# andrenarchy/krypy

Hardware: AMD Instinct MI355X
Metric: GMRES iterations/sec + SpMV HBM GB/s, n=10^7 5-pt Laplacian fp64 (higher is better)
Workload: dtype f64; 1 GPU; GMRES(100) restart cycles, 2-D 5-pt Laplacian 4000x2500 CSR (N=10000000, nnz=49987000), b=rng(0) normal, x0=0, tol=1e-8 (BASELINE.json configs[1]); n=10000000, ortho=mgs, restart=100, parallelism=1 GPU, ranks=1

## Files before the change

krypy_amd/csrc/chain.h:

```cpp
#pragma once
#include <type_traits>
#include "kernels.h"

namespace kh {

constexpr int CH_BS = 512;
constexpr int CH_GMAX = 512;

struct ChainArgs {
    int64_t n2;
    int64_t chunk2;
    const double* V;
    const double* B;
    int64_t ld;
    int64_t col0;
    int ncol;
    int sweeps;
    const double* w_in;
    const double* dg;
    double* vnext;
    double* pnext;
    double* hdev;
    int64_t hnext;
    unsigned long long* gran;
// ... 631 lines not shown
#pragma unroll
    for (int d = 0; d < FND; ++d) {
#pragma unroll
        for (int p = 0; p < 2; ++p) {
            const int o = a.offs.off[d] + p;
            kq[d][p] = (unsigned)((o >> 1) - g.lo * CH_BS);
            kh[d][p] = (o & 1) ? H : 0u;
        }
    }
    {
        const int64_t b0 = first + (int64_t)g.lo * CH_BS;
        constexpr int PG = 8;
#pragma unroll
        for (int j0 = 0; j0 < NWB - 1; j0 += PG) {
            double2 t[PG];
#pragma unroll
            for (int j = j0; j < j0 + PG && j < NWB - 1; ++j) t[j - j0] = xw.load(b0 + (int64_t)(j < spanb ? j : spanb - 1) * CH_BS);
            CH_ISSUE_FENCE();
#pragma unroll
            for (int j = j0; j < j0 + PG && j < NWB - 1; ++j) xw.store((unsigned)j, tid, t[j - j0]);
        }
    }
    double2 st[D];
    unsigned mk[D];
    int64_t fb = first;
    const int64_t hs = (int64_t)(g.hi + 1) * CH_BS;
#pragma unroll
    for (int r = 0; r < D; ++r) {
        mk[r] = dia_mask_load(a.dmask, fb + (int64_t)r * CH_BS);
        st[r] = xw.load(fb + hs + (int64_t)r * CH_BS);
    }
    unsigned sl = (unsigned)spanb;
    unsigned tb = (unsigned)tid;
    ch_lds_barrier();
#pragma unroll
    for (int r = 0; r < R2; ++r) {
        const unsigned m = mk[r % D];
        const unsigned pos = (unsigned)((r % NWB) * CH_BS) + tb;
        double2 av[FND];
        double x0[FND], x1[FND];
#pragma unroll
        for (int d = 0; d < FND; ++d) {
            av[d] = dia_slot<true>(a.dia, a.dia_ld, d, 0, m, a.offs.cst[d]);
            x0[d] = xw.get(pos, kq[d][0], kh[d][0]);
            x1[d] = xw.get(pos, kq[d][1], kh[d][1]);
        }
        double s0 = 0.0, s1 = 0.0;
#pragma unroll
        for (int d = 0; d < FND; ++d) {
            const double p0 = av[d].x * x0[d], p1 = av[d].y * x1[d];
            s0 = (av[d].x != 0.0) ? s0 + p0 : s0;
            s1 = (av[d].y != 0.0) ? s1 + p1 : s1;
        }
        put(r, s0, s1);
        if (r + 1 < R2) {
            xw.store(sl, tid, st[r % D]);
            sl = (sl + 1 == (unsigned)NWB) ? 0u : sl + 1;
        }
        if (r + D < R2) mk[r % D] = dia_mask_load(a.dmask, fb + (int64_t)(r + D) * CH_BS);
        if (r + D + 1 < R2) st[r % D] = xw.load(fb + hs + (int64_t)(r + D) * CH_BS);
        ch_lds_barrier();
        asm volatile("" : "+v"(fb), "+v"(tb) : : "memory");
    }
}

template <int R2, int FND, int RIF = KH_RIF, class Put>
__device__ __forceinline__ void chain_apply_banded(const ChainArgs& a, int64_t first, Put&& put) {
    static_assert(FND <= KH_DIA_CMAX, "the mask form holds up to KH_DIA_CMAX diagonals");
    if (a.dmask != nullptr) chain_apply_banded_form<R2, FND, RIF, true>(a, first, put);
    else chain_apply_banded_form<R2, FND, RIF, false>(a, first, put);
}

template <int R2, bool MASKED, bool CPLX = false, int FND = 0, int WL = 0, bool ONEX = false, bool XR = false>
__global__ __launch_bounds__(CH_BS) void k_mgs_chain(ChainArgs a) {
    static_assert(FND == 0 || !MASKED, "the fused operator exists for the padded kernels");
    static_assert(!XR || (!CPLX && !ONEX), "the cross-rank stage exists for real vectors spread over the chip");
    constexpr int RW = R2 - WL;
    extern __shared__ __attribute__((aligned(16))) double2 wl[];
#define W_GET(r) (((r) < RW) ? w[((r) < RW) ? (r) : 0] : wl[((r) - RW) * CH_BS + tid])
#define W_PUT(r, val)                                   \
    do {                                                \
        if ((r) < RW) w[((r) < RW) ? (r) : 0] = (val);  \
        else wl[((r) - RW) * CH_BS + tid] = (val);      \
    } while (0)
    constexpr int PB = ChainShape<R2>::PB;
    constexpr int NB = ChainShape<R2>::NB;
    __shared__ double smd[4 * (CH_BS / 64)];
    __shared__ unsigned smu[2 * CH_GMAX];
    __shared__ int slead;
    const int tid = threadIdx.x;
    int G = gridDim.x;
    int bid = blockIdx.x;
    GridRole role;
    if constexpr (ONEX) {
        if (!onex_enter(a, &slead, bid, G, role)) return;
    } else {
        role = grid_role(a.xcc_leader, a.epoch0, &slead);
    }
    const int64_t first = (int64_t)bid * a.chunk2 + tid;
    const int64_t left = a.n2 - first;
    const int rem = (int)(left < 0 ? 0 : (left > a.chunk2 ? a.chunk2 : left));
#define CH_OK(r) (!MASKED || (r) * CH_BS < rem)
    double2 w[RW];
    double2 ring[2][PB];
    if constexpr (FND > 0 && CPLX) {
        chain_apply_banded_z<R2, FND>(a, first, [&](int r, double s0, double s1) { W_PUT(r, make_double2(s0, s1)); });
    } else if constexpr (FND > 0) {
        chain_apply_banded<R2, FND>(a, first, [&](int r, double s0, double s1) { W_PUT(r, make_double2(s0, s1)); });
    } else {
        const double2* __restrict__ win2 = reinterpret_cast<const double2*>(a.w_in) + first;
#pragma unroll
        for (int r = 0; r < R2; ++r) {
            const double2 v = win2[(int64_t)r * CH_BS];
            double2 t;
            t.x = CH_OK(r) ? v.x : 0.0;
            t.y = CH_OK(r) ? v.y : 0.0;
            W_PUT(r, t);
            if ((r + 1) % 8 == 0) CH_ISSUE_FENCE();
        }
    }
    if (a.presub) {
        const double hk = (a.h_km1_dev != nullptr) ? a.h_km1_dev[0] : a.h_km1;
        const double2* __restrict__ p2 = reinterpret_cast<const double2*>(a.bprev) + first;
#pragma unroll
        for (int r = 0; r < R2; ++r) {
            const double2 p = p2[(int64_t)r * CH_BS];
            double2 t = W_GET(r);
            t.x = CH_OK(r) ? t.x - hk * p.x : 0.0;
            t.y = CH_OK(r) ? t.y - hk * p.y : 0.0;
            W_PUT(r, t);
            if ((r + 1) % 8 == 0) CH_ISSUE_FENCE();
        }
    }
    unsigned epoch = a.epoch0;
    if (a.debug == 4 && tid == 0) __hip_atomic_store(a.err, 1, __ATOMIC_RELAXED, __HIP_MEMORY_SCOPE_AGENT);
    const int total = a.ncol * a.sweeps;
    {
        const double2* __restrict__ v2 = reinterpret_cast<const double2*>(a.V + a.col0 * a.ld) + first;
#pragma unroll
        for (int i = 0; i < PB; ++i) ring[0][i] = v2[(int64_t)i * CH_BS];
        CH_ISSUE_FENCE();
    }
    for (int t = 0; t < total; ++t) {
        const int64_t j = a.col0 + (t % a.ncol);
        const double2* __restrict__ v2 = reinterpret_cast<const double2*>(a.V + j * a.ld) + first;
        const double2* __restrict__ b2 = reinterpret_cast<const double2*>(a.B + j * a.ld) + first;
        double acc0 = 0.0, acc1 = 0.0;
        if (a.debug != 2)
#pragma unroll
        for (int b = 0; b < NB; ++b) {
            const double2* __restrict__ nx = (b + 1 < NB) ? v2 + (int64_t)(b + 1) * PB * CH_BS : b2;
#pragma unroll
            for (int i = 0; i < PB; ++i)
                ring[(b + 1) & 1][i] = (WL > 0 && b + 1 == NB) ? ld_nt2(nx + (int64_t)i * CH_BS) : nx[(int64_t)i * CH_BS];
            CH_ISSUE_FENCE();
#pragma unroll
            for (int i = 0; i < PB; ++i) {
                double2 v = ring[b & 1][i];
                if (MASKED && !CH_OK(b * PB + i)) v = make_double2(0.0, 0.0);
                const double2 wr = W_GET(b * PB + i);
                if (CPLX) {
                    acc0 = fma(v.x, wr.x, acc0);
                    acc0 = fma(v.y, wr.y, acc0);
                    acc1 = fma(v.x, wr.y, acc1);
                    acc1 = fma(-v.y, wr.x, acc1);
                } else {
                    acc0 = fma(v.x, wr.x, acc0);
                    acc1 = fma(v.y, wr.y, acc1);
                }
            }
        }
        double alpha, alpha_i = 0.0;
        if (CPLX) {
            alpha = acc0;
            alpha_i = acc1;
            if constexpr (ONEX) {
                double pv[2] = {alpha, alpha_i};
                onex_sum<2>(pv, epoch++, a.gran, G, bid, a.err, smd);
                alpha = pv[0];
                alpha_i = pv[1];
            } else {
                grid_sum2(alpha, alpha_i, epoch++, a.gran, G, a.err, smd, smu, role, a.xcc_res);
            }
            if (bid == 0 && tid == 0) {
                a.hdev[2 * j] = (t < a.ncol ? 0.0 : a.hdev[2 * j]) + alpha;
                a.hdev[2 * j + 1] = (t < a.ncol ? 0.0 : a.hdev[2 * j + 1]) + alpha_i;
            }
        } else {
            if constexpr (ONEX) {
                double pv[1] = {acc0 + acc1};
                onex_sum<1>(pv, epoch++, a.gran, G, bid, a.err, smd);
                alpha = pv[0];
            } else {
                const unsigned e_ = epoch++;
                alpha = (a.debug == 1) ? (acc0 + acc1) * 1e-30
                                       : grid_sum<XR>(acc0 + acc1, e_, a.gran, G, a.err, smd, smu, role, a.xcc_res, nullptr, &a.xr,
                                                      a.xr.epoch0 + (e_ - a.epoch0));
            }
            if (bid == 0 && tid == 0) a.hdev[j] = (t < a.ncol ? 0.0 : a.hdev[j]) + alpha;
        }
        if (a.debug == 4) alpha *= 0.5;
        const int64_t jn = a.col0 + ((t + 1) % a.ncol);
        const double2* __restrict__ vn = (t + 1 < total)
            ? reinterpret_cast<const double2*>(a.V + jn * a.ld) + first
            : reinterpret_cast<const double2*>(a.w_in) + first;
        if (a.debug != 2)
#pragma unroll
        for (int b = 0; b < NB; ++b) {
            const double2* __restrict__ nx = (b + 1 < NB) ? b2 + (int64_t)(b + 1) * PB * CH_BS : vn;
#pragma unroll
            for (int i = 0; i < PB; ++i)
                ring[(b + 1) & 1][i] = (WL > 0 && b + 1 < NB) ? ld_nt2(nx + (int64_t)i * CH_BS) : nx[(int64_t)i * CH_BS];
            CH_ISSUE_FENCE();
#pragma unroll
            for (int i = 0; i < PB; ++i) {
                const double2 p = ring[b & 1][i];
                const int r = b * PB + i;
                double2 wr = W_GET(r);
                if (CPLX) {
                    const double tr = alpha * p.x - alpha_i * p.y;
                    const double ti = alpha * p.y + alpha_i * p.x;
                    wr.x = CH_OK(r) ? wr.x - tr : 0.0;
                    wr.y = CH_OK(r) ? wr.y - ti : 0.0;
                } else {
                    wr.x = CH_OK(r) ? wr.x - alpha * p.x : 0.0;
                    wr.y = CH_OK(r) ? wr.y - alpha * p.y : 0.0;
                }
                W_PUT(r, wr);
            }
        }
    }
    double acc = 0.0;
    if (a.dg != nullptr) {
        const double2* __restrict__ d2 = reinterpret_cast<const double2*>(a.dg) + first;
#pragma unroll
        for (int r = 0; r < R2; ++r) {
            const double2 d = d2[(int64_t)r * CH_BS];
            const double2 wr = W_GET(r);
            acc = fma(wr.x, d.x * wr.x, acc);
            acc = fma(wr.y, d.y * wr.y, acc);
            if ((r + 1) % 8 == 0) CH_ISSUE_FENCE();
        }
    } else {
#pragma unroll
        for (int r = 0; r < R2; ++r) {
            const double2 wr = W_GET(r);
            acc = fma(wr.x, wr.x, acc);
            acc = fma(wr.y, wr.y, acc);
        }
    }
    double h2;
    if constexpr (ONEX) {
        double pv[1] = {acc};
        onex_sum<1>(pv, epoch++, a.gran, G, bid, a.err, smd);
        h2 = pv[0];
    } else {
        const unsigned e_ = epoch++;
        h2 = grid_sum<XR>(acc, e_, a.gran, G, a.err, smd, smu, role, a.xcc_res, nullptr, &a.xr, a.xr.epoch0 + (e_ - a.epoch0));
    }
    const double h = sqrt(fabs(h2));
    if (bid == 0 && tid == 0) a.hdev[a.hnext] = h;
    double2* __restrict__ vn2 = reinterpret_cast<double2*>(a.vnext) + first;
    if (a.dg != nullptr) {
        double2* __restrict__ pn2 = reinterpret_cast<double2*>(a.pnext) + first;
        const double2* __restrict__ d2 = reinterpret_cast<const double2*>(a.dg) + first;
#pragma unroll
        for (int r = 0; r < R2; ++r) {
            if (r * CH_BS < rem) {
                const double2 d = d2[(int64_t)r * CH_BS];
                const double2 wr = W_GET(r);
                double2 o, m;
                o.x = wr.x / h;
                o.y = wr.y / h;
                m.x = (d.x * wr.x) / h;
                m.y = (d.y * wr.y) / h;
                st_nt2(pn2 + (int64_t)r * CH_BS, o);
                st_nt2(vn2 + (int64_t)r * CH_BS, m);
            }
        }
    } else {
#pragma unroll
        for (int r = 0; r < R2; ++r) {
            if (r * CH_BS < rem) {
                const double2 wr = W_GET(r);
                double2 o;
                o.x = wr.x / h;
                o.y = wr.y / h;
                st_nt2(vn2 + (int64_t)r * CH_BS, o);
            }
        }
    }
    if (bid == 0 && a.hpin != nullptr) {
        __syncthreads();
        for (int i = tid; i < a.hcount; i += CH_BS)
            a.hpin[i] = __hip_atomic_load(a.hdev + i, __ATOMIC_RELAXED, __HIP_MEMORY_SCOPE_AGENT);
        if (tid == 0) *a.errpin = __hip_atomic_load(a.err, __ATOMIC_RELAXED, __HIP_MEMORY_SCOPE_AGENT);
        CH_SIGNAL_DONE(a);
    }
#undef W_PUT
#undef W_GET
#undef CH_OK
}

#ifndef KH_CH_REUSE_SKIP
#define KH_CH_REUSE_SKIP 0
#endif
#ifndef KH_CH_SKIP_LAST
#define KH_CH_SKIP_LAST 0
#endif
#ifndef KH_CH_LDS_EARLY
#define KH_CH_LDS_EARLY 0
#endif
#ifndef KH_XWIN_AHEAD
#define KH_XWIN_AHEAD 4
#endif
template <int R2, bool CPLX = false>
struct ChainShapeLds {
    static constexpr int PB = ChainShape<R2>::PB;
    static constexpr int NB = R2 / PB;
    static constexpr int WL = (R2 == 40 && !CPLX) ? 4 : 0;
    static constexpr int LROWS = (R2 == 40 && !CPLX) ? 19 : (NB >= 4 ? 3 : 1) * PB;
    static constexpr int NG = NB - 1 - LROWS / PB;
    static_assert((NB % 2) == 0 && NG >= 0 && (NG % 2) == 0, "ring parity must reset every phase");
    static_assert(WL <= LROWS && LROWS <= R2 - PB, "the prologue's rows of w borrow parked rows; the last batch stays in the ring");
    static constexpr size_t LDS_BYTES = (size_t)LROWS * CH_BS * sizeof(double2);
    static constexpr int XWIN_BLOCKS = LROWS - WL;
    static constexpr size_t STATIC_LDS = 4 * (CH_BS / 64) * sizeof(double) + 2 * CH_GMAX * sizeof(unsigned) + sizeof(int);
    static_assert(LDS_BYTES + STATIC_LDS <= 160 * 1024, "a CU has 160 KB of LDS");
};

template <int R2, bool MASKED, bool CPLX = false, int FND = 0, bool XR = false>
__global__ __launch_bounds__(CH_BS) void k_mgs_chain_lds(ChainArgs a) {
    static_assert(FND == 0 || !MASKED, "the fused operator exists for the padded kernels");
    static_assert(!XR || !CPLX, "the cross-rank stage exists for real vectors");
    constexpr int PB = ChainShapeLds<R2, CPLX>::PB;
    constexpr int NB = ChainShapeLds<R2, CPLX>::NB;
    constexpr int LROWS = ChainShapeLds<R2, CPLX>::LROWS;
    constexpr int LBC = (LROWS + PB - 1) / PB;
    constexpr bool SPLIT = (LROWS % PB) != 0;
    constexpr int NG = ChainShapeLds<R2, CPLX>::NG;
    constexpr int WL = FND > 0 ? ChainShapeLds<R2, CPLX>::WL : 0;
    constexpr int RW = R2 - WL;
    extern __shared__ __attribute__((aligned(16))) double2 vlds[];
#define W_GET_N(r, NR) (((r) < (NR)) ? w[((r) < (NR)) ? (r) : 0] : vlds[((r) - (NR)) * CH_BS + tid])
#define W_PUT_N(r, val, NR)                                 \
    do {                                                    \
        if ((r) < (NR)) w[((r) < (NR)) ? (r) : 0] = (val);  \
        else vlds[((r) - (NR)) * CH_BS + tid] = (val);      \
    } while (0)
#define W_GET(r) W_GET_N(r, RW)
#define W_PUT(r, val) W_PUT_N(r, val, RW)
    __shared__ double smd[4 * (CH_BS / 64)];
    __shared__ unsigned smu[2 * CH_GMAX];
    __shared__ int slead;
    const int tid = threadIdx.x;
    const int G = gridDim.x;
    const GridRole role = grid_role(a.xcc_leader, a.epoch0, &slead);
    const int64_t first = (int64_t)blockIdx.x * a.chunk2 + tid;
    const int64_t left = a.n2 - first;
    const int rem = (int)(left < 0 ? 0 : (left > a.chunk2 ? a.chunk2 : left));
#define CH_OK(r) (!MASKED || (r) * CH_BS < rem)
#define CH_LD(ptr, reuse) ((reuse) ? *(ptr) : ld_nt2(ptr))
    double2 w[R2];
    double2 ring[2][PB];
    if constexpr (FND > 0 && CPLX) {
        chain_apply_banded_z<R2, FND>(a, first, [&](int r, double s0, double s1) { W_PUT(r, make_double2(s0, s1)); });
    } else if constexpr (FND > 0 && !XR) {
        constexpr int NWB = ChainShapeLds<R2, CPLX>::XWIN_BLOCKS;
        if (a.xwin)
            chain_apply_banded_xwin<R2, FND, NWB, KH_XWIN_AHEAD>(a, first, reinterpret_cast<double*>(vlds + WL * CH_BS),
                                                                 [&](int r, double s0, double s1) { W_PUT(r, make_double2(s0, s1)); });
        else
            chain_apply_banded<R2, FND>(a, first, [&](int r, double s0, double s1) { W_PUT(r, make_double2(s0, s1)); });
    } else if constexpr (FND > 0) {
        chain_apply_banded<R2, FND>(a, first, [&](int r, double s0, double s1) { W_PUT(r, make_double2(s0, s1)); });
    } else {
        const double2* __restrict__ win2 = reinterpret_cast<const double2*>(a.w_in) + first;
#pragma unroll
        for (int r = 0; r < R2; ++r) {
            const double2 v = ld_nt2(win2 + (int64_t)r * CH_BS);
            double2 t;
            t.x = CH_OK(r) ? v.x : 0.0;
            t.y = CH_OK(r) ? v.y : 0.0;
            W_PUT(r, t);
            if ((r + 1) % 8 == 0) CH_ISSUE_FENCE();
        }
    }
    if (a.presub) {
        const double hk = (a.h_km1_dev != nullptr) ? a.h_km1_dev[0] : a.h_km1;
        const double2* __restrict__ p2 = reinterpret_cast<const double2*>(a.bprev) + first;
#pragma unroll
        for (int r = 0; r < R2; ++r) {
            const double2 p = p2[(int64_t)r * CH_BS];
            double2 t = W_GET(r);
            t.x = CH_OK(r) ? t.x - hk * p.x : 0.0;
            t.y = CH_OK(r) ? t.y - hk * p.y : 0.0;
            W_PUT(r, t);
            if ((r + 1) % 8 == 0) CH_ISSUE_FENCE();
        }
    }
    if constexpr (WL > 0) {
#pragma unroll
        for (int r = RW; r < R2; ++r) w[r] = vlds[(r - RW) * CH_BS + tid];
        CH_ISSUE_FENCE();
    }
#undef W_PUT
#undef W_GET
#define W_GET(r) W_GET_N(r, R2)
#define W_PUT(r, val) W_PUT_N(r, val, R2)
    unsigned epoch = a.epoch0;
    if (a.debug == 4 && tid == 0) __hip_atomic_store(a.err, 1, __ATOMIC_RELAXED, __HIP_MEMORY_SCOPE_AGENT);
    const int total = a.ncol * a.sweeps;
    {
        const double2* __restrict__ v2 = reinterpret_cast<const double2*>(a.V + a.col0 * a.ld) + first;
#pragma unroll
        for (int i = 0; i < PB; ++i) ring[0][i] = CH_LD(v2 + (int64_t)i * CH_BS, false);
        CH_ISSUE_FENCE();
    }
#if defined(KH_CHAIN_TRACE) && KH_CHAIN_TRACE == 2
    unsigned long long tr_acc[9] = {0, 0, 0, 0, 0, 0, 0, 0, 0};
#endif
    for (int t = 0; t < total; ++t) {
        const int64_t j = a.col0 + (t % a.ncol);
        const double2* __restrict__ v2 = reinterpret_cast<const double2*>(a.V + j * a.ld) + first;
        const int64_t jn = a.col0 + ((t + 1) % a.ncol);
        const double2* __restrict__ vn = (t + 1 < total)
            ? reinterpret_cast<const double2*>(a.V + jn * a.ld) + first
            : reinterpret_cast<const double2*>(a.w_in) + first;
        double acc0 = 0.0, acc1 = 0.0;
        CH_STAMP(a, t, total, 0);
#pragma unroll
        for (int b = 0; b < NB; ++b) {
            const double2* __restrict__ nx = (b + 1 < NB) ? v2 + (int64_t)(b + 1) * PB * CH_BS
                                                            : (NG > 0 ? v2 + (int64_t)(NB - 2) * PB * CH_BS : vn);
#pragma unroll
            for (int i = 0; i < PB; ++i) {
                if (!SPLIT || b + 1 < NB || NG == 0 || (NB - 2) * PB + i >= LROWS)
                    ring[(b + 1) & 1][i] = CH_LD(nx + (int64_t)i * CH_BS, (b + 1 < NB) && (!SPLIT || (b + 1) * PB + i >= LROWS) &&
                                                                              (b + 1 >= LROWS / PB + KH_CH_REUSE_SKIP) && (b + 1 <= NB - 2 - KH_CH_SKIP_LAST));
            }
            CH_ISSUE_FENCE();
#pragma unroll
            for (int i = 0; i < PB; ++i) {
                double2 v = ring[b & 1][i];
                if (MASKED && !CH_OK(b * PB + i)) v = make_double2(0.0, 0.0);
                if (SPLIT ? (b * PB + i < LROWS) : (b < LBC)) vlds[(b * PB + i) * CH_BS + tid] = v;
                const double2 wr = W_GET(b * PB + i);
                if (CPLX) {
                    acc0 = fma(v.x, wr.x, acc0);
                    acc0 = fma(v.y, wr.y, acc0);
                    acc1 = fma(v.x, wr.y, acc1);
                    acc1 = fma(-v.y, wr.x, acc1);
                } else {
                    acc0 = fma(v.x, wr.x, acc0);
                    acc1 = fma(v.y, wr.y, acc1);
                }
            }
        }
        double alpha, alpha_i = 0.0;
        CH_STAMP(a, t, total, 1);
        if (CPLX) {
            alpha = acc0;
            alpha_i = acc1;
            grid_sum2(alpha, alpha_i, epoch++, a.gran, G, a.err, smd, smu, role, a.xcc_res);
            if (blockIdx.x == 0 && tid == 0) {
                a.hdev[2 * j] = (t < a.ncol ? 0.0 : a.hdev[2 * j]) + alpha;
                a.hdev[2 * j + 1] = (t < a.ncol ? 0.0 : a.hdev[2 * j + 1]) + alpha_i;
            }
        } else {
#if defined(KH_CHAIN_TRACE) && KH_CHAIN_TRACE == 2
            alpha = grid_sum(acc0 + acc1, epoch++, a.gran, G, a.err, smd, smu, role, a.xcc_res, tr_acc);
#elif defined(KH_CHAIN_TRACE)
            alpha = grid_sum(acc0 + acc1, epoch++, a.gran, G, a.err, smd, smu, role, a.xcc_res,
                             a.trace ? a.trace + (((size_t)blockIdx.x * total) + t) * 16 : nullptr);
#else
            const unsigned e_ = epoch++;
            alpha = (a.debug == 1) ? (acc0 + acc1) * 1e-30
                                   : grid_sum<XR>(acc0 + acc1, e_, a.gran, G, a.err, smd, smu, role, a.xcc_res, nullptr, &a.xr,
                                                  a.xr.epoch0 + (e_ - a.epoch0));
#endif
            if (blockIdx.x == 0 && tid == 0) a.hdev[j] = (t < a.ncol ? 0.0 : a.hdev[j]) + alpha;
        }
        if (a.debug == 4) alpha *= 0.5;
        CH_STAMP(a, t, total, 5);
#define CH_UPD(r, p)                                              \
    do {                                                          \
        double2 wr_ = W_GET(r);                                   \
        if (CPLX) {                                               \
            const double tr = alpha * (p).x - alpha_i * (p).y;    \
            const double ti = alpha * (p).y + alpha_i * (p).x;    \
            wr_.x = CH_OK(r) ? wr_.x - tr : 0.0;                  \
            wr_.y = CH_OK(r) ? wr_.y - ti : 0.0;                  \
        } else {                                                  \
            wr_.x = CH_OK(r) ? wr_.x - alpha * (p).x : 0.0;       \
            wr_.y = CH_OK(r) ? wr_.y - alpha * (p).y : 0.0;       \
        }                                                         \
        W_PUT(r, wr_);                                            \
    } while (0)
#pragma unroll
        for (int i = 0; i < PB; ++i) CH_UPD((NB - 1) * PB + i, ring[1][i]);
        constexpr bool EARLY = (KH_CH_LDS_EARLY != 0) && NG >= 2;
#pragma unroll
        for (int g = 0; g < NG; ++g) {
            const int b = NB - 2 - g;
            const double2* __restrict__ nx = (g + 1 < NG) ? v2 + (int64_t)(b - 1) * PB * CH_BS : vn;
#pragma unroll
            for (int i = 0; i < PB; ++i) {
                if (!SPLIT || g + 1 == NG || (b - 1) * PB + i >= LROWS) ring[(g + 1) & 1][i] = CH_LD(nx + (int64_t)i * CH_BS, false);
            }
            CH_ISSUE_FENCE();
            if (EARLY && g == 1) {
#pragma unroll
                for (int bb = LBC - 1; bb >= 0; --bb) {
#pragma unroll
                    for (int i = 0; i < PB; ++i) {
                        if (!SPLIT || bb * PB + i < LROWS) {
                            const double2 p = vlds[(bb * PB + i) * CH_BS + tid];
                            CH_UPD(bb * PB + i, p);
                        }
                    }
                    CH_ISSUE_FENCE();
                }
            }
#pragma unroll
            for (int i = 0; i < PB; ++i) {
                if (!SPLIT || b * PB + i >= LROWS) CH_UPD(b * PB + i, ring[g & 1][i]);
            }
        }
        CH_STAMP(a, t, total, 6);
        if (!EARLY) {
#pragma unroll
            for (int b = LBC - 1; b >= 0; --b) {
                CH_ISSUE_FENCE();
#pragma unroll
                for (int i = 0; i < PB; ++i) {
                    if (!SPLIT || b * PB + i < LROWS) {
                        const double2 p = vlds[(b * PB + i) * CH_BS + tid];
                        CH_UPD(b * PB + i, p);
                    }
                }
            }
        }
#undef CH_UPD
        CH_STAMP(a, t, total, 7);
    }
#if defined(KH_CHAIN_TRACE) && KH_CHAIN_TRACE == 2
    if (a.trace != nullptr && (tid == 0 || tid == CH_BS - 64)) {
#pragma unroll
        for (int i = 0; i < 8; ++i) a.trace[((size_t)blockIdx.x * 2 + (tid ? 1 : 0)) * 8 + i] = tr_acc[i];
    }
#endif
    double acc = 0.0;
    if (a.dg != nullptr) {
        const double2* __restrict__ d2 = reinterpret_cast<const double2*>(a.dg) + first;
#pragma unroll
        for (int r = 0; r < R2; ++r) {
            const double2 d = d2[(int64_t)r * CH_BS];
            const double2 wr = W_GET(r);
            acc = fma(wr.x, d.x * wr.x, acc);
            acc = fma(wr.y, d.y * wr.y, acc);
            if ((r + 1) % 8 == 0) CH_ISSUE_FENCE();
        }
    } else {
#pragma unroll
        for (int r = 0; r < R2; ++r) {
            const double2 wr = W_GET(r);
            acc = fma(wr.x, wr.x, acc);
            acc = fma(wr.y, wr.y, acc);
        }
    }
    const unsigned en_ = epoch++;
    const double h2 = grid_sum<XR>(acc, en_, a.gran, G, a.err, smd, smu, role, a.xcc_res, nullptr, &a.xr, a.xr.epoch0 + (en_ - a.epoch0));
    const double h = sqrt(fabs(h2));
    if (blockIdx.x == 0 && tid == 0) a.hdev[a.hnext] = h;
    double2* __restrict__ vn2 = reinterpret_cast<double2*>(a.vnext) + first;
    if (a.dg != nullptr) {
        double2* __restrict__ pn2 = reinterpret_cast<double2*>(a.pnext) + first;
        const double2* __restrict__ d2 = reinterpret_cast<const double2*>(a.dg) + first;
#pragma unroll
        for (int r = 0; r < R2; ++r) {
            if (r * CH_BS < rem) {
                const double2 d = d2[(int64_t)r * CH_BS];
                const double2 wr = W_GET(r);
                double2 o, m;
                o.x = wr.x / h;
                o.y = wr.y / h;
                m.x = (d.x * wr.x) / h;
                m.y = (d.y * wr.y) / h;
                st_nt2(pn2 + (int64_t)r * CH_BS, o);
                st_nt2(vn2 + (int64_t)r * CH_BS, m);
            }
        }
    } else {
#pragma unroll
        for (int r = 0; r < R2; ++r) {
            if (r * CH_BS < rem) {
                const double2 wr = W_GET(r);
                double2 o;
                o.x = wr.x / h;
                o.y = wr.y / h;
                st_nt2(vn2 + (int64_t)r * CH_BS, o);
            }
        }
    }
    if (blockIdx.x == 0 && a.hpin != nullptr) {
        __syncthreads();
        for (int i = tid; i < a.hcount; i += CH_BS)
            a.hpin[i] = __hip_atomic_load(a.hdev + i, __ATOMIC_RELAXED, __HIP_MEMORY_SCOPE_AGENT);
        if (tid == 0) *a.errpin = __hip_atomic_load(a.err, __ATOMIC_RELAXED, __HIP_MEMORY_SCOPE_AGENT);
        CH_SIGNAL_DONE(a);
    }
#undef W_PUT
#undef W_GET
#undef W_PUT_N
#undef W_GET_N
#undef CH_LD
#undef CH_OK
}

template <int R2>
struct ChainShapePf {
    static constexpr int PB = ChainShape<R2>::PB;
    static constexpr int NB = R2 / PB;
    static constexpr int LB = (NB - 2 < 3) ? NB - 2 : 3;
    static constexpr int NG = NB - 2 - LB;
    static_assert((NB % 2) == 0 && NB >= 2 && LB >= 0 && NG >= 0 && NG <= LB, "shape");
    static constexpr int ROW_BYTES = CH_BS * (int)sizeof(double2);
    static constexpr int STATIC_LDS = 2 * (CH_BS / 64) * 8 + 2 * CH_GMAX * 4 + 256;
    static constexpr int SPARE = (160 * 1024 - STATIC_LDS - LB * PB * ROW_BYTES) / ROW_BYTES;
#ifndef KH_PF_SP_CAP
#define KH_PF_SP_CAP 64
#endif
    static constexpr int SP0 = SPARE < PB ? SPARE : PB;
    static constexpr int SP = SP0 < KH_PF_SP_CAP ? SP0 : KH_PF_SP_CAP;
    static_assert(SP0 >= 1, "at least one spare row");
    static constexpr size_t LDS_BYTES = (size_t)(LB * PB + SP) * ROW_BYTES;
};

typedef __attribute__((address_space(3))) double2 ch_lds_double2;

__device__ __forceinline__ void ch_dma16(const double2* gsrc, unsigned lds_dst) {
    unsigned keep;
    asm volatile("s_mov_b32 %0, m0\n\ts_mov_b32 m0, %2\n\ts_nop 0\n\tglobal_load_lds_dwordx4 %1, off\n\ts_mov_b32 m0, %0"
                 : "=&s"(keep)
                 : "v"(gsrc), "s"(lds_dst)
                 : "memory");
}

template <int R2, bool MASKED, bool CPLX = false, int FND = 0, bool ONEX = false>
__global__ __launch_bounds__(CH_BS) void k_mgs_chain_pf(ChainArgs a) {
    static_assert(FND == 0 || (!MASKED && !CPLX), "the fused operator exists for the padded real kernel");
    constexpr int PB = ChainShapePf<R2>::PB;
    constexpr int NB = ChainShapePf<R2>::NB;
    constexpr int LB = ChainShapePf<R2>::LB;
    constexpr int NG = ChainShapePf<R2>::NG;
    constexpr int SP = ChainShapePf<R2>::SP;
    extern __shared__ __attribute__((aligned(16))) double2 vlds[];
    double2* const vsp = vlds + (size_t)LB * PB * CH_BS;
    __shared__ double smd[4 * (CH_BS / 64)];
    __shared__ unsigned smu[2 * CH_GMAX];
    __shared__ int slead;
    const int tid = threadIdx.x;
    int G = gridDim.x;
    int bid = blockIdx.x;
    GridRole role;
    if constexpr (ONEX) {
        if (!onex_enter(a, &slead, bid, G, role)) return;
    } else {
        role = grid_role(a.xcc_leader, a.epoch0, &slead);
    }
    const int64_t first = (int64_t)bid * a.chunk2 + tid;
    const int64_t left = a.n2 - first;
    const int rem = (int)(left < 0 ? 0 : (left > a.chunk2 ? a.chunk2 : left));
    const unsigned lds_wave = (unsigned)(size_t)((ch_lds_double2*)vlds) +
                              (unsigned)__builtin_amdgcn_readfirstlane((tid >> 6) * 64 * (int)sizeof(double2));
#define CH_OK(r) (!MASKED || (r) * CH_BS < rem)
#define CH_LD(ptr, reuse) ((reuse) ? *(ptr) : ld_nt2(ptr))
    double2 w[R2];
    double2 ring[2][PB];
    if constexpr (FND > 0) {
        chain_apply_banded<R2, FND>(a, first, [&](int r, double s0, double s1) { w[r] = make_double2(s0, s1); });
    } else {
        const double2* __restrict__ win2 = reinterpret_cast<const double2*>(a.w_in) + first;
#pragma unroll
        for (int r = 0; r < R2; ++r) {
            const double2 v = ld_nt2(win2 + (int64_t)r * CH_BS);
            w[r].x = CH_OK(r) ? v.x : 0.0;
            w[r].y = CH_OK(r) ? v.y : 0.0;
            if ((r + 1) % 8 == 0) CH_ISSUE_FENCE();
        }
    }
    if (a.presub) {
        const double hk = (a.h_km1_dev != nullptr) ? a.h_km1_dev[0] : a.h_km1;
        const double2* __restrict__ p2 = reinterpret_cast<const double2*>(a.bprev) + first;
#pragma unroll
        for (int r = 0; r < R2; ++r) {
            const double2 p = p2[(int64_t)r * CH_BS];
            w[r].x = CH_OK(r) ? w[r].x - hk * p.x : 0.0;
            w[r].y = CH_OK(r) ? w[r].y - hk * p.y : 0.0;
            if ((r + 1) % 8 == 0) CH_ISSUE_FENCE();
        }
    }
    unsigned epoch = a.epoch0;
    if (a.debug == 4 && tid == 0) __hip_atomic_store(a.err, 1, __ATOMIC_RELAXED, __HIP_MEMORY_SCOPE_AGENT);
    const int total = a.ncol * a.sweeps;
#define CH_REUSE(b) ((b) >= LB && (b) < LB + NG)
    {
        const double2* __restrict__ v2 = reinterpret_cast<const double2*>(a.V + a.col0 * a.ld) + first;
#pragma unroll
        for (int i = 0; i < SP; ++i)
            ch_dma16(v2 + (int64_t)i * CH_BS, lds_wave + (unsigned)(((LB * PB + i) * CH_BS) * sizeof(double2)));
#pragma unroll
        for (int i = SP; i < PB; ++i) ring[0][i] = CH_LD(v2 + (int64_t)i * CH_BS, CH_REUSE(0));
        CH_ISSUE_FENCE();
        if (NB > 1) {
#pragma unroll
            for (int i = 0; i < PB; ++i) ring[1][i] = CH_LD(v2 + (int64_t)(PB + i) * CH_BS, CH_REUSE(1));
            CH_ISSUE_FENCE();
        }
    }
    for (int t = 0; t < total; ++t) {
        const int64_t j = a.col0 + (t % a.ncol);
        const double2* __restrict__ v2 = reinterpret_cast<const double2*>(a.V + j * a.ld) + first;
        const int64_t jn = a.col0 + ((t + 1) % a.ncol);
        const double2* __restrict__ vn = (t + 1 < total)
            ? reinterpret_cast<const double2*>(a.V + jn * a.ld) + first
            : reinterpret_cast<const double2*>(a.w_in) + first;
        double acc0 = 0.0, acc1 = 0.0;
        asm volatile("s_waitcnt vmcnt(%0)" ::"n"(2 * PB - SP) : "memory");
#pragma unroll
        for (int b = 0; b < NB; ++b) {
#pragma unroll
            for (int i = 0; i < PB; ++i) {
                double2 v = (b == 0 && i < SP) ? vsp[i * CH_BS + tid] : ring[b & 1][i];
                if (MASKED && !CH_OK(b * PB + i)) v = make_double2(0.0, 0.0);
                if (NB == 2 && b == 0 && i < SP) ring[0][i] = v;
                if (b < LB) vlds[(b * PB + i) * CH_BS + tid] = v;
                if (CPLX) {
                    acc0 = fma(v.x, w[b * PB + i].x, acc0);
                    acc0 = fma(v.y, w[b * PB + i].y, acc0);
                    acc1 = fma(v.x, w[b * PB + i].y, acc1);
                    acc1 = fma(-v.y, w[b * PB + i].x, acc1);
                } else {
                    acc0 = fma(v.x, w[b * PB + i].x, acc0);
                    acc1 = fma(v.y, w[b * PB + i].y, acc1);
                }
            }
            if (b + 2 < NB) {
                CH_ISSUE_FENCE();
#pragma unroll
                for (int i = 0; i < PB; ++i)
                    ring[b & 1][i] = CH_LD(v2 + (int64_t)((b + 2) * PB + i) * CH_BS, CH_REUSE(b + 2));
                CH_ISSUE_FENCE();
            }
        }
        asm volatile("s_waitcnt lgkmcnt(0)" ::: "memory");
#pragma unroll
        for (int i = 0; i < SP; ++i)
            ch_dma16(vn + (int64_t)i * CH_BS, lds_wave + (unsigned)(((LB * PB + i) * CH_BS) * sizeof(double2)));
        double alpha, alpha_i = 0.0;
        if (CPLX) {
            alpha = acc0;
            alpha_i = acc1;
            if constexpr (ONEX) {
                double pv[2] = {alpha, alpha_i};
                onex_sum<2>(pv, epoch++, a.gran, G, bid, a.err, smd);
                alpha = pv[0];
                alpha_i = pv[1];
            } else {
                grid_sum2(alpha, alpha_i, epoch++, a.gran, G, a.err, smd, smu, role, a.xcc_res);
            }
            if (bid == 0 && tid == 0) {
                a.hdev[2 * j] = (t < a.ncol ? 0.0 : a.hdev[2 * j]) + alpha;
                a.hdev[2 * j + 1] = (t < a.ncol ? 0.0 : a.hdev[2 * j + 1]) + alpha_i;
            }
        } else {
            if constexpr (ONEX) {
                double pv[1] = {acc0 + acc1};
                onex_sum<1>(pv, epoch++, a.gran, G, bid, a.err, smd);
                alpha = pv[0];
            } else {
                alpha = (a.debug == 1) ? (acc0 + acc1) * 1e-30
                                       : grid_sum(acc0 + acc1, epoch++, a.gran, G, a.err, smd, smu, role, a.xcc_res);
            }
            if (bid == 0 && tid == 0) a.hdev[j] = (t < a.ncol ? 0.0 : a.hdev[j]) + alpha;
        }
        if (a.debug == 4) alpha *= 0.5;
#define CH_UPD(r, p)                                              \
    do {                                                          \
        if (CPLX) {                                               \
            const double tr = alpha * (p).x - alpha_i * (p).y;    \
            const double ti = alpha * (p).y + alpha_i * (p).x;    \
            w[r].x = CH_OK(r) ? w[r].x - tr : 0.0;                \
            w[r].y = CH_OK(r) ? w[r].y - ti : 0.0;                \
        } else {                                                  \
            w[r].x = CH_OK(r) ? w[r].x - alpha * (p).x : 0.0;     \
            w[r].y = CH_OK(r) ? w[r].y - alpha * (p).y : 0.0;     \
        }                                                         \
    } while (0)
#pragma unroll
        for (int b = 0; b < LB; ++b) {
            CH_ISSUE_FENCE();
#pragma unroll
            for (int i = 0; i < PB; ++i) {
                const double2 p = vlds[(b * PB + i) * CH_BS + tid];
                CH_UPD(b * PB + i, p);
            }
        }
        if constexpr (NG > 0) {
            asm volatile("s_waitcnt lgkmcnt(0)" ::: "memory");
#pragma unroll
            for (int g = 0; g < NG; ++g)
#pragma unroll
                for (int i = 0; i < PB; ++i)
                    ch_dma16(v2 + (int64_t)((LB + g) * PB + i) * CH_BS,
                             lds_wave + (unsigned)(((g * PB + i) * CH_BS) * sizeof(double2)));
        }
        if (NB > 1) {
#pragma unroll
            for (int i = 0; i < PB; ++i) CH_UPD((NB - 2) * PB + i, ring[0][i]);
            CH_ISSUE_FENCE();
#pragma unroll
            for (int i = SP; i < PB; ++i) ring[0][i] = CH_LD(vn + (int64_t)i * CH_BS, CH_REUSE(0));
            CH_ISSUE_FENCE();
#pragma unroll
            for (int i = 0; i < PB; ++i) CH_UPD((NB - 1) * PB + i, ring[1][i]);
            CH_ISSUE_FENCE();
#pragma unroll
            for (int i = 0; i < PB; ++i) ring[1][i] = CH_LD(vn + (int64_t)(PB + i) * CH_BS, CH_REUSE(1));
            CH_ISSUE_FENCE();
        }
        if constexpr (NG > 0) {
            asm volatile("s_waitcnt vmcnt(%0)" ::"n"(2 * PB - SP) : "memory");
#pragma unroll
            for (int g = 0; g < NG; ++g) {
                CH_ISSUE_FENCE();
#pragma unroll
                for (int i = 0; i < PB; ++i) {
                    const double2 p = vlds[(g * PB + i) * CH_BS + tid];
                    CH_UPD((LB + g) * PB + i, p);
                }
            }
        }
#undef CH_UPD
    }
// ... 464 lines not shown
```

Baseline: 1240 iterations/s.

## Hold last two register batches across MGS chain and prefetch two steps ahead

```diff
diff --git a/krypy_amd/csrc/chain.h b/krypy_amd/csrc/chain.h
--- a/krypy_amd/csrc/chain.h
+++ b/krypy_amd/csrc/chain.h
@@ -957,6 +957,10 @@
 #undef CH_OK
 }
 
+#ifndef KH_CH_HOLD2
+#define KH_CH_HOLD2 2
+#endif
+static_assert(KH_CH_HOLD2 >= 0 && KH_CH_HOLD2 <= 2, "KH_CH_HOLD2: 0 (the earlier schedule), 1 or 2");
 #ifndef KH_CH_REUSE_SKIP
 #define KH_CH_REUSE_SKIP 0
 #endif
@@ -976,7 +980,8 @@
     static constexpr int WL = (R2 == 40 && !CPLX) ? 4 : 0;
     static constexpr int LROWS = (R2 == 40 && !CPLX) ? 19 : (NB >= 4 ? 3 : 1) * PB;
     static constexpr int NG = NB - 1 - LROWS / PB;
-    static_assert((NB % 2) == 0 && NG >= 0 && (NG % 2) == 0, "ring parity must reset every phase");
+    static_assert((NB % 2) == 0 && NG >= 0, "the dot phase starts in ring[0] and must end with batch NB-1 in ring[1]");
+    static_assert(KH_CH_HOLD2 != 0 || (NG % 2) == 0, "KH_CH_HOLD2 = 0: NG ring steps from ring[0] on must end in ring[0]");
     static_assert(WL <= LROWS && LROWS <= R2 - PB, "the prologue's rows of w borrow parked rows; the last batch stays in the ring");
     static constexpr size_t LDS_BYTES = (size_t)LROWS * CH_BS * sizeof(double2);
     static constexpr int XWIN_BLOCKS = LROWS - WL;
@@ -994,6 +999,8 @@
     constexpr int LBC = (LROWS + PB - 1) / PB;
     constexpr bool SPLIT = (LROWS % PB) != 0;
     constexpr int NG = ChainShapeLds<R2, CPLX>::NG;
+    constexpr bool HOLD2 = (KH_CH_HOLD2 != 0) && NG > 0;
+    constexpr int RLAST = HOLD2 ? NB - 3 : NB - 2;
     constexpr int WL = FND > 0 ? ChainShapeLds<R2, CPLX>::WL : 0;
     constexpr int RW = R2 - WL;
     extern __shared__ __attribute__((aligned(16))) double2 vlds[];
@@ -1090,9 +1097,10 @@
                                                             : (NG > 0 ? v2 + (int64_t)(NB - 2) * PB * CH_BS : vn);
 #pragma unroll
             for (int i = 0; i < PB; ++i) {
+                if (HOLD2 && b + 1 == NB) continue;
                 if (!SPLIT || b + 1 < NB || NG == 0 || (NB - 2) * PB + i >= LROWS)
                     ring[(b + 1) & 1][i] = CH_LD(nx + (int64_t)i * CH_BS, (b + 1 < NB) && (!SPLIT || (b + 1) * PB + i >= LROWS) &&
-                                                                              (b + 1 >= LROWS / PB + KH_CH_REUSE_SKIP) && (b + 1 <= NB - 2 - KH_CH_SKIP_LAST));
+                                                                              (b + 1 >= LROWS / PB + KH_CH_REUSE_SKIP) && (b + 1 <= RLAST - KH_CH_SKIP_LAST));
             }
             CH_ISSUE_FENCE();
 #pragma unroll
@@ -1152,6 +1160,56 @@
         }                                                         \
         W_PUT(r, wr_);                                            \
     } while (0)
+#define CH_UPD_HEAD()                                                         \
+    do {                                                                      \
+        _Pragma("unroll") for (int bb = LBC - 1; bb >= 0; --bb) {             \
+            CH_ISSUE_FENCE();                                                 \
+            _Pragma("unroll") for (int i = 0; i < PB; ++i) {                  \
+                if (!SPLIT || bb * PB + i < LROWS) {                          \
+                    const double2 p = vlds[(bb * PB + i) * CH_BS + tid];      \
+                    CH_UPD(bb * PB + i, p);                                   \
+                }                                                             \
+            }                                                                 \
+        }                                                                     \
+        CH_ISSUE_FENCE();                                                     \
+    } while (0)
+        if constexpr (HOLD2) {
+#pragma unroll
+            for (int i = 0; i < PB; ++i) CH_UPD((NB - 1) * PB + i, ring[1][i]);
+#pragma unroll
+            for (int i = 0; i < PB; ++i) CH_UPD((NB - 2) * PB + i, ring[0][i]);
+            constexpr int MS = NG - 1;
+            constexpr int VP = (KH_CH_HOLD2 == 2 || MS == 0) ? MS : MS - 1;
+#define CH_H2_ISSUE(p_)                                                                                                   \
+    do {                                                                                                                  \
+        if ((p_) == VP) {                                                                                                 \
+            _Pragma("unroll") for (int i = 0; i < PB; ++i) ring[0][i] = CH_LD(vn + (int64_t)i * CH_BS, false);            \
+        } else {                                                                                                          \
+            const int bq_ = NB - 3 - ((p_) < VP ? (p_) : (p_) - 1);                                                       \
+            _Pragma("unroll") for (int i = 0; i < PB; ++i) {                                                              \
+                if (!SPLIT || bq_ * PB + i >= LROWS)                                                                      \
+                    ring[((p_) + VP) & 1][i] = CH_LD(v2 + (int64_t)(bq_ * PB + i) * CH_BS, false);                        \
+            }                                                                                                             \
+        }                                                                                                                 \
+        CH_ISSUE_FENCE();                                                                                                 \
+    } while (0)
+            CH_H2_ISSUE(0);
+            if (MS >= 1) CH_H2_ISSUE(1);
+            if (KH_CH_LDS_EARLY != 0) CH_UPD_HEAD();
+#pragma unroll
+            for (int s = 0; s < MS; ++s) {
+                const int p = s < VP ? s : s + 1;
+                const int b = NB - 3 - s;
+#pragma unroll
+                for (int i = 0; i < PB; ++i) {
+                    if (!SPLIT || b * PB + i >= LROWS) CH_UPD(b * PB + i, ring[(p + VP) & 1][i]);
+                }
+                if (p + 2 <= MS) CH_H2_ISSUE(p + 2);
+            }
+#undef CH_H2_ISSUE
+            CH_STAMP(a, t, total, 6);
+            if (KH_CH_LDS_EARLY == 0) CH_UPD_HEAD();
+        } else {
 #pragma unroll
         for (int i = 0; i < PB; ++i) CH_UPD((NB - 1) * PB + i, ring[1][i]);
         constexpr bool EARLY = (KH_CH_LDS_EARLY != 0) && NG >= 2;
@@ -1196,6 +1254,8 @@
                 }
             }
         }
+        }
+#undef CH_UPD_HEAD
 #undef CH_UPD
         CH_STAMP(a, t, total, 7);
     }
```

Result: faster. 1274 iterations/s (median of 6 runs) (+2.8%).
